# google-research/hyperbo

Measured on AMD Instinct MI355X. Metric: GP NLL+grad evals/sec at N=8192 D=16 fp64, higher is better.
Workload: dtype f64

## Files before the change

### hyperbo_amd/csrc/gemm.hip

```cpp
#include "hbo_internal.h"

namespace {

template <typename T> struct Mma;
template <> struct Mma<double> {
  typedef double acc_t __attribute__((ext_vector_type(4)));
  typedef double vec_t __attribute__((ext_vector_type(2)));
  static __device__ __forceinline__ acc_t mma(double a, double b, acc_t c) {
    return __builtin_amdgcn_mfma_f64_16x16x4f64(a, b, c, 0, 0, 0);
  }
  static __device__ __forceinline__ int crow(int lane, int r) { return (lane >> 4) + 4 * r; }
};
template <> struct Mma<float> {
  typedef float acc_t __attribute__((ext_vector_type(4)));
  typedef float vec_t __attribute__((ext_vector_type(4)));
  static __device__ __forceinline__ acc_t mma(float a, float b, acc_t c) {
    return __builtin_amdgcn_mfma_f32_16x16x4f32(a, b, c, 0, 0, 0);
  }
  static __device__ __forceinline__ int crow(int lane, int r) { return 4 * (lane >> 4) + r; }
};

template <typename T> __device__ __host__ constexpr int skc() { return sizeof(T) == 8 ? 17 : 36; }
template <int TM> __device__ __host__ constexpr int smc() { return TM + 16; }
constexpr int OPERAND_BYTES = 18432;
constexpr int OPERAND_BYTES_64 = 10240;
constexpr int GEMM_LDS_BYTES_64 = 4 * OPERAND_BYTES_64;
constexpr int GEMM_LDS_BYTES = 4 * OPERAND_BYTES;

template <typename T, bool KC, int TM>
__device__ __forceinline__ T frag_read(const T* s, int mn, int k) {
  return KC ? s[mn * skc<T>() + k] : s[k * smc<TM>() + mn];
}

template <typename T>
struct TileJob {
  const T* A; int64_t lda;
  const T* B; int64_t ldb;
  T* C; int64_t ldc;
  T* colsq;
  int ksteps;
  T alpha;
  int beta;
  int* yield_flag;
};

template <typename T, int TM>
__device__ __forceinline__ bool decode_job(const GemmArgs& g, TileJob<T>& j, const int bxi, const int byi, const int gdx, const int task) {
  constexpr int BKE = 128 / sizeof(T);
  const TaskDesc& t = g.tasks[task];
  const int64_t ld = t.ld;
  const int nblk = t.nblk;
  j.colsq = nullptr;
  switch (g.mode) {
    case GEMM_SYRK: {
      constexpr int U = HBO_TILE / TM;
      const int by = byi;
      const int bx = gridDim.z > 1 ? (int)((bxi + 5 * byi + 3 * task) % gdx) : bxi;
      const int c = g.c_lo * U + by;
      const int r = g.c_lo * U + bx;
      const int nrt = (nblk + ((g.aug & 1) ? 1 : 0)) * U;
      const int chi = (g.c_hi < nblk ? g.c_hi : nblk) * U;
      if (c >= chi || r < c || r >= nrt) return false;
      T* Am = static_cast<T*>(t.A);
      j.A = Am + (int64_t)r * TM * ld + (int64_t)g.p0 * HBO_TILE;
      j.B = Am + (int64_t)c * TM * ld + (int64_t)g.p0 * HBO_TILE;
      j.C = Am + (int64_t)r * TM * ld + (int64_t)c * TM;
      j.lda = j.ldb = j.ldc = ld;
      j.ksteps = g.kt * HBO_TILE / BKE;
      j.alpha = (T)-1; j.beta = 1;
#ifdef HBO_GEMM_DEBUG
      if (g.aug & 2) j.beta = 0;
      if (g.aug & 4) { j.C = nullptr; j.beta = 0; }
#endif
      return true;
    }
    case GEMM_TRTRI_A:
    case GEMM_TRTRI_B: {
      constexpr int U = HBO_TILE / TM;
      const int s = g.p0, su = s * U;
      const int grp = g.grp_lo + bxi / su;
      const int inner = bxi % su;
      int jt, it;
      if (g.mode == GEMM_TRTRI_A) {
        jt = byi;
        const int vu = (grp == g.c_hi ? g.c_lo : s) * U;
        it = (inner + 5 * byi + 3 * task) % vu;
      }
      else { it = (g.kt > 0 ? g.kt * U : su) - 1 - byi; jt = inner; }
      const int64_t o = (int64_t)grp * 2 * s * HBO_TILE;
      const int64_t R = o + (int64_t)s * HBO_TILE + (int64_t)it * TM;
      if (R >= (int64_t)nblk * HBO_TILE) return false;
      const int64_t Cc = o + (int64_t)jt * TM;
      const T* L = static_cast<const T*>(t.A);
      T* W = static_cast<T*>(t.W);
      T* S = static_cast<T*>(t.S);
      if (g.mode == GEMM_TRTRI_A) {
        j.A = L + R * ld + Cc;
        j.B = W + Cc * ld + Cc;
        j.C = S + R * ld + Cc;
        j.ksteps = (s * HBO_TILE - jt * TM) / BKE;
        j.alpha = (T)1;
      } else {
        const int64_t o2 = o + (int64_t)s * HBO_TILE;
        j.A = W + R * ld + o2;
        j.B = S + o2 * ld + Cc;
        j.C = W + R * ld + Cc;
        j.ksteps = (it + 1) * TM / BKE;
        j.alpha = (T)-1;
      }
      j.lda = j.ldb = j.ldc = ld;
      j.beta = 0;
      return true;
    }
    case GEMM_LAUUM: {
      constexpr int U = HBO_TILE / TM;
      int i, jt;
      if (U == 1) {
        int lin = bxi;
        if (lin >= nblk * (nblk + 1) / 2) return false;
        i = 0;
        while (lin > i) { lin -= i + 1; ++i; }
        jt = lin;
      } else {
        int lin = bxi;
        if (lin >= 2 * nblk * (nblk + 1)) return false;
        i = 0;
        while (lin > (i | 1)) { lin -= (i | 1) + 1; ++i; }
        jt = lin;
      }
      const int64_t k0 = (int64_t)i * TM;
      const T* W = static_cast<const T*>(t.W);
      j.A = W + k0 * ld + (int64_t)i * TM;
      j.B = W + k0 * ld + (int64_t)jt * TM;
      j.C = static_cast<T*>(t.S) + (int64_t)i * TM * ld + (int64_t)jt * TM;
      j.lda = j.ldb = j.ldc = ld;
      j.ksteps = (int)(((int64_t)nblk * HBO_TILE - k0) / BKE);
      j.alpha = (T)1; j.beta = 0;
      return true;
    }
    case GEMM_SWEEP_B: {
      constexpr int U = HBO_TILE / TM;
      const int b0 = g.c_lo, b1 = g.c_hi < nblk ? g.c_hi : nblk;
      const int rows = (b1 - b0) * U;
      if (byi >= rows || bxi >= b0 * U) return false;
      const int it = b0 * U + rows - 1 - byi, jt = bxi;
      const int64_t k0 = (int64_t)b0 * HBO_TILE;
      T* W = static_cast<T*>(t.W);
      j.A = W + (int64_t)it * TM * ld + k0;
      j.B = static_cast<const T*>(t.S) + k0 * ld + (int64_t)jt * TM;
      j.C = W + (int64_t)it * TM * ld + (int64_t)jt * TM;
      j.lda = j.ldb = j.ldc = ld;
      j.ksteps = (int)(((int64_t)(it + 1) * TM - k0) / BKE);
      j.alpha = (T)-1; j.beta = 0;
      return true;
    }
    case GEMM_SWEEP_T: {
      constexpr int U = HBO_TILE / TM;
      const int b0 = g.c_lo, b1 = g.c_hi;
      if (b1 >= nblk) return false;
      const int below = (nblk - b1) * U;
      const int bx = gridDim.z > 1 || g.ptasks > 1 ? (int)((bxi + 5 * byi + 3 * task) % gdx) : bxi;
      if (bx >= below || byi >= b1 * U) return false;
      const int it = b1 * U + bx, jt = byi;
      const int64_t kb = (int64_t)b0 * HBO_TILE, kj = (int64_t)jt * TM;
      const int64_t k0 = kj > kb ? kj : kb;
      j.A = static_cast<const T*>(t.A) + (int64_t)it * TM * ld + k0;
      j.B = static_cast<const T*>(t.W) + k0 * ld + kj;
      j.C = static_cast<T*>(t.S) + (int64_t)it * TM * ld + kj;
      j.lda = j.ldb = j.ldc = ld;
      j.ksteps = (int)(((int64_t)b1 * HBO_TILE - k0) / BKE);
      j.alpha = (T)1; j.beta = kj >= kb ? 0 : 1;
      return true;
    }
    case GEMM_SWEEP_C: {
      constexpr int U = HBO_TILE / TM;
      const int b0 = g.c_lo, b1 = g.c_hi < nblk ? g.c_hi : nblk;
      if (b1 <= b0) return false;
      int i = 0, lin = bxi, jt;
      if (U == 1) {
        if (lin >= b1 * (b1 + 1) / 2) return false;
        while (lin > i) { lin -= i + 1; ++i; }
      } else {
        if (lin >= 2 * b1 * (b1 + 1)) return false;
        while (lin > (i | 1)) { lin -= (i | 1) + 1; ++i; }
      }
      jt = lin;
      const int64_t kb = (int64_t)b0 * HBO_TILE, ki = (int64_t)i * TM;
      const int64_t k0 = ki > kb ? ki : kb;
      const T* W = static_cast<const T*>(t.W);
      j.A = W + k0 * ld + ki;
      j.B = W + k0 * ld + (int64_t)jt * TM;
      j.C = static_cast<T*>(t.S) + ki * ld + (int64_t)jt * TM;
      j.lda = j.ldb = j.ldc = ld;
      j.ksteps = (int)(((int64_t)b1 * HBO_TILE - k0) / BKE);
      j.alpha = (T)1; j.beta = ki >= kb ? 0 : 1;
      return true;
    }
    case GEMM_VTV: {
      const T* Vm = static_cast<const T*>(g.B);
      j.A = Vm + (int64_t)byi * HBO_TILE;
      j.B = Vm + (int64_t)bxi * HBO_TILE;
      j.C = static_cast<T*>(g.V) + (int64_t)byi * HBO_TILE * g.ldb + (int64_t)bxi * HBO_TILE;
      j.lda = j.ldb = j.ldc = g.ldb;
      j.ksteps = nblk * HBO_TILE / BKE;
      j.alpha = (T)-1; j.beta = 1;
      return true;
    }
    case GEMM_POST: {
      if (g.kchunk > 0) {
        int i = 0, rem = byi;
        for (;; ++i) {
          if (i >= nblk) return false;
          const int nch = (i + g.kchunk) / g.kchunk;
          if (rem < nch) break;
          rem -= nch;
        }
        const int k0 = rem * g.kchunk;
        const int kb = (i + 1 - k0 < g.kchunk ? i + 1 - k0 : g.kchunk);
        const T* W = static_cast<const T*>(t.W);
        j.A = W + (int64_t)i * HBO_TILE * ld + (int64_t)k0 * HBO_TILE;
        j.lda = ld;
        j.B = static_cast<const T*>(g.B) + (int64_t)k0 * HBO_TILE * g.ldb + (int64_t)bxi * HBO_TILE;
        j.ldb = g.ldb;
        j.C = static_cast<T*>(g.V) + ((int64_t)rem * nblk * HBO_TILE + (int64_t)i * HBO_TILE) * g.ldb + (int64_t)bxi * HBO_TILE;
        j.ldc = g.ldb;
        j.ksteps = kb * HBO_TILE / BKE;
        j.alpha = (T)1; j.beta = 0;
        return true;
      }
      const int i = nblk - 1 - byi;
      if (i < 0) return false;
      const int jq = bxi;
      const T* W = static_cast<const T*>(t.W);
      j.A = W + (int64_t)i * HBO_TILE * ld;
      j.lda = ld;
      j.B = static_cast<const T*>(g.B) + (int64_t)jq * HBO_TILE;
      j.ldb = g.ldb;
      j.C = g.V ? static_cast<T*>(g.V) + (int64_t)i * HBO_TILE * g.ldb + (int64_t)jq * HBO_TILE : nullptr;
      j.ldc = g.ldb;
      j.colsq = g.colsq ? static_cast<T*>(g.colsq) + (int64_t)i * g.ldb + (int64_t)jq * HBO_TILE : nullptr;
      j.ksteps = (i + 1) * HBO_TILE / BKE;
      j.alpha = (T)1; j.beta = 0;
      return true;
    }
  }
  return false;
}

template <typename T>
__device__ __forceinline__ unsigned long long uniform_addr(const T* p) {
  const unsigned long long v = reinterpret_cast<unsigned long long>(p);
  const unsigned lo = __builtin_amdgcn_readfirstlane((unsigned)v), hi = __builtin_amdgcn_readfirstlane((unsigned)(v >> 32));
  return ((unsigned long long)hi << 32) | lo;
}
__device__ __forceinline__ __amdgpu_buffer_rsrc_t tile_rsrc(unsigned long long addr) {
  return __builtin_amdgcn_make_buffer_rsrc(reinterpret_cast<void*>(addr), 0, 0x7fffffff, 0x00020000);
}
template <typename T, bool KC, int TM>
__device__ __forceinline__ void stage_offsets(int64_t ld, int (&off)[TM / 32], int tid) {
  constexpr int VEC = 16 / sizeof(T);
  if (KC) {
    const int c = tid & 7, row = tid >> 3;
#pragma unroll
    for (int q = 0; q < TM / 32; ++q) off[q] = (int)(((int64_t)(row + 32 * q) * ld + c * VEC) * (int64_t)sizeof(T));
  } else {
    constexpr int CPR = TM / VEC, RPP = 256 / CPR;
    const int c = tid % CPR, kr = tid / CPR;
#pragma unroll
    for (int q = 0; q < TM / 32; ++q) off[q] = (int)(((int64_t)(kr + RPP * q) * ld + c * VEC) * (int64_t)sizeof(T));
  }
}
template <typename T>
__device__ __forceinline__ typename Mma<T>::vec_t piece_load(unsigned long long slab, int off) {
  return __builtin_bit_cast(typename Mma<T>::vec_t, __builtin_amdgcn_raw_buffer_load_b128(tile_rsrc(slab), off, 0, 0));
}
template <typename T, bool KC, int TM>
__device__ __forceinline__ void piece_store(T* s, const typename Mma<T>::vec_t& r, int q, int tid) {
  typedef typename Mma<T>::vec_t vec_t;
  constexpr int VEC = 16 / sizeof(T);
  if (KC) {
    const int c = tid & 7, row = tid >> 3;
    if ((skc<T>() * sizeof(T)) % 16 == 0) {
      *reinterpret_cast<vec_t*>(s + (row + 32 * q) * skc<T>() + c * VEC) = r;
    } else {
#pragma unroll
      for (int e = 0; e < VEC; ++e) s[(row + 32 * q) * skc<T>() + c * VEC + e] = r[e];
    }
  } else {
    constexpr int CPR = TM / VEC, RPP = 256 / CPR;
    const int c = tid % CPR, kr = tid / CPR;
    *reinterpret_cast<vec_t*>(s + (kr + RPP * q) * smc<TM>() + c * VEC) = r;
  }
}

template <typename T, bool AKC, bool BKC, int TM>
__device__ __forceinline__ void gemm_tile2(const TileJob<T>& job, unsigned char* smem) {
  typedef typename Mma<T>::acc_t acc_t;
  typedef typename Mma<T>::vec_t vec_t;
  constexpr int BKE = 128 / sizeof(T);
  constexpr int KK = BKE / 4;
  constexpr int MI = TM / 32;
  constexpr int WT = TM / 2;
  static_assert(MI == 4 && KK >= 4 && KK % 2 == 0, "the interleave below is written for the 128-tile: 16 MFMAs and 8 fragments per k step, 8 pieces per slab");
  T* sA = reinterpret_cast<T*>(smem);
  T* sB = reinterpret_cast<T*>(smem + OPERAND_BYTES);
  const int tid = threadIdx.x, lane = tid & 63, wave = tid >> 6;
  const int wm = wave >> 1, wn = wave & 1;
  const int l15 = lane & 15, lq = lane >> 4;

  acc_t acc[MI][MI];
  if (job.beta) {
    const T inv_alpha = (T)1 / job.alpha;
#pragma unroll
    for (int a = 0; a < MI; ++a)
#pragma unroll
      for (int b = 0; b < MI; ++b)
#pragma unroll
        for (int r = 0; r < 4; ++r) {
          const int row = wm * WT + a * 16 + Mma<T>::crow(lane, r);
          const int col = wn * WT + b * 16 + l15;
          acc[a][b][r] = gld(job.C + (int64_t)row * job.ldc + col) * inv_alpha;
        }
  } else {
#pragma unroll
    for (int a = 0; a < MI; ++a)
#pragma unroll
      for (int b = 0; b < MI; ++b) acc[a][b] = (acc_t){0, 0, 0, 0};
  }

  const int nk = job.ksteps;
  int offa[MI], offb[MI];
  stage_offsets<T, AKC, TM>(job.lda, offa, tid);
  stage_offsets<T, BKC, TM>(job.ldb, offb, tid);
  unsigned long long slabA = uniform_addr(job.A), slabB = uniform_addr(job.B);
  const unsigned long long stepA = uniform_addr(reinterpret_cast<const char*>((AKC ? (int64_t)BKE : (int64_t)BKE * job.lda) * (int64_t)sizeof(T)));
  const unsigned long long stepB = uniform_addr(reinterpret_cast<const char*>((BKC ? (int64_t)BKE : (int64_t)BKE * job.ldb) * (int64_t)sizeof(T)));
  vec_t ra[MI], rb[MI];
#pragma unroll
  for (int q = 0; q < MI; ++q) { ra[q] = piece_load<T>(slabA, offa[q]); rb[q] = piece_load<T>(slabB, offb[q]); }
#pragma unroll
  for (int q = 0; q < MI; ++q) { piece_store<T, AKC, TM>(sA, ra[q], q, tid); piece_store<T, BKC, TM>(sB, rb[q], q, tid); }
  if (nk > 1) { slabA += stepA; slabB += stepB; }
#pragma unroll
  for (int q = 0; q < MI; ++q) { ra[q] = piece_load<T>(slabA, offa[q]); rb[q] = piece_load<T>(slabB, offb[q]); }
  __syncthreads();

  T af[2][MI], bf[2][MI];
#define HBO_SB() __builtin_amdgcn_sched_barrier(0)
  auto frag = [&](int set, int kk, int i) {
    const int k = kk * 4 + lq;
    if (i < MI) af[set][i] = frag_read<T, AKC, TM>(sA, wm * WT + i * 16 + l15, k);
    else bf[set][i - MI] = frag_read<T, BKC, TM>(sB, wn * WT + (i - MI) * 16 + l15, k);
  };
  auto mma = [&](int set, int i) {
    const int a = i / MI, b = (a & 1) ? MI - 1 - i % MI : i % MI;
    acc[a][b] = Mma<T>::mma(af[set][a], bf[set][b], acc[a][b]);
  };
  auto step_reads = [&](int set, int nset, int nkk) {
#pragma unroll
    for (int i = 0; i < 16; ++i) {
      mma(set, i);
      if (i < 4) { HBO_SB(); frag(nset, nkk, 2 * i); frag(nset, nkk, 2 * i + 1); HBO_SB(); }
    }
  };
  auto piece_out = [&](int j) {
    if (j < MI) piece_store<T, AKC, TM>(sA, ra[j], j, tid); else piece_store<T, BKC, TM>(sB, rb[j - MI], j - MI, tid);
  };
  auto piece_in = [&](int j) {
    if (j < MI) ra[j] = piece_load<T>(slabA, offa[j]); else rb[j - MI] = piece_load<T>(slabB, offb[j - MI]);
  };
#pragma unroll
  for (int i = 0; i < 2 * MI; ++i) frag(0, 0, i);

  const int* const yslot = job.yield_flag ? job.yield_flag + cu_token() : nullptr;
  int ypoll = 0;
  for (int kt = 0; kt + 1 < nk; ++kt) {
    if (yslot) {
      if (ypoll != 0)
        for (int spin = 0; spin < 256 && __hip_atomic_load(yslot, __ATOMIC_RELAXED, __HIP_MEMORY_SCOPE_AGENT) != 0; ++spin)
          __builtin_amdgcn_s_sleep(16);
      ypoll = __hip_atomic_load(yslot, __ATOMIC_RELAXED, __HIP_MEMORY_SCOPE_AGENT);
    }
    if (kt + 2 < nk) { slabA += stepA; slabB += stepB; }
#pragma unroll
    for (int kk = 0; kk < KK - 2; ++kk) step_reads(kk & 1, (kk + 1) & 1, kk + 1);
#pragma unroll
    for (int i = 0; i < 7; ++i) {
      mma(0, i);
      if (i < 4) { HBO_SB(); frag(1, KK - 1, 2 * i); frag(1, KK - 1, 2 * i + 1); HBO_SB(); }
    }
    HBO_SB(); __syncthreads(); HBO_SB();
    mma(0, 7);
#pragma unroll
    for (int j = 0; j < 4; ++j) {
      HBO_SB(); piece_out(j); HBO_SB(); mma(0, 8 + 2 * j); HBO_SB(); piece_in(j); HBO_SB(); mma(0, 9 + 2 * j);
    }
#pragma unroll
    for (int j = 4; j < 8; ++j) {
      HBO_SB(); piece_out(j); HBO_SB(); mma(1, 2 * (j - 4)); HBO_SB(); piece_in(j); HBO_SB(); mma(1, 2 * (j - 4) + 1);
    }
    mma(1, 8); mma(1, 9);
    HBO_SB(); __syncthreads(); HBO_SB();
    mma(1, 10);
#pragma unroll
    for (int i = 0; i < 4; ++i) { HBO_SB(); frag(0, 0, 2 * i); frag(0, 0, 2 * i + 1); HBO_SB(); mma(1, 11 + i); }
    mma(1, 15);
    HBO_SB();
  }
#pragma unroll
  for (int kk = 0; kk < KK - 1; ++kk) step_reads(kk & 1, (kk + 1) & 1, kk + 1);
#pragma unroll
  for (int i = 0; i < 16; ++i) mma(1, i);
#undef HBO_SB
  if (yslot) __syncthreads();

  if (job.C) {
#pragma unroll
    for (int a = 0; a < MI; ++a)
#pragma unroll
      for (int b = 0; b < MI; ++b)
#pragma unroll
        for (int r = 0; r < 4; ++r) {
          const int row = wm * WT + a * 16 + Mma<T>::crow(lane, r);
          const int col = wn * WT + b * 16 + l15;
          gst(job.C + (int64_t)row * job.ldc + col, job.alpha * acc[a][b][r]);
        }
  }
  if (TM == 128 && job.colsq) {
    __syncthreads();
    T* red = reinterpret_cast<T*>(smem);
    T part[MI];
#pragma unroll
    for (int b = 0; b < MI; ++b) {
      T s_ = 0;
#pragma unroll
      for (int a = 0; a < MI; ++a)
#pragma unroll
        for (int r = 0; r < 4; ++r) s_ += acc[a][b][r] * acc[a][b][r];
      s_ += __shfl_xor(s_, 16);
      s_ += __shfl_xor(s_, 32);
      part[b] = s_;
    }
    if (lq == 0) {
#pragma unroll
      for (int b = 0; b < MI; ++b) red[wave * 64 + b * 16 + l15] = part[b];
    }
    __syncthreads();
    if (tid < 128) {
      const int wn2 = tid >> 6, c = tid & 63;
      gst(job.colsq + wn2 * 64 + c, red[(0 * 2 + wn2) * 64 + c] + red[(1 * 2 + wn2) * 64 + c]);
    }
  }
}
constexpr int PF64 = 2;
constexpr int LB64 = 4;
template <typename T, bool AKC, bool BKC, int TM, int PF>
__device__ __forceinline__ void gemm_tile3(const TileJob<T>& job, unsigned char* smem) {
  typedef typename Mma<T>::acc_t acc_t;
  typedef typename Mma<T>::vec_t vec_t;
  constexpr int BKE = 128 / sizeof(T);
  constexpr int KK = BKE / 4;
  constexpr int MI = TM / 32;
  constexpr int WT = TM / 2;
  static_assert(MI == 2 && KK >= 4 && KK % 2 == 0, "written for the 64-tile: 4 MFMAs and 4 fragments per k step, 4 pieces per slab");
  T* sA = reinterpret_cast<T*>(smem);
  T* sB = reinterpret_cast<T*>(smem + OPERAND_BYTES_64);
  const int tid = threadIdx.x, lane = tid & 63, wave = tid >> 6;
  const int wm = wave >> 1, wn = wave & 1;
  const int l15 = lane & 15, lq = lane >> 4;

  acc_t acc[MI][MI];
  if (job.beta) {
    const T inv_alpha = (T)1 / job.alpha;
#pragma unroll
    for (int a = 0; a < MI; ++a)
#pragma unroll
      for (int b = 0; b < MI; ++b)
#pragma unroll
        for (int r = 0; r < 4; ++r) {
          const int row = wm * WT + a * 16 + Mma<T>::crow(lane, r);
          const int col = wn * WT + b * 16 + l15;
          acc[a][b][r] = gld(job.C + (int64_t)row * job.ldc + col) * inv_alpha;
        }
  } else {
#pragma unroll
    for (int a = 0; a < MI; ++a)
#pragma unroll
      for (int b = 0; b < MI; ++b) acc[a][b] = (acc_t){0, 0, 0, 0};
  }

  const int nk = job.ksteps;
  int offa[MI], offb[MI];
  stage_offsets<T, AKC, TM>(job.lda, offa, tid);
  stage_offsets<T, BKC, TM>(job.ldb, offb, tid);
  unsigned long long slabA = uniform_addr(job.A), slabB = uniform_addr(job.B);
  const unsigned long long stepA = uniform_addr(reinterpret_cast<const char*>((AKC ? (int64_t)BKE : (int64_t)BKE * job.lda) * (int64_t)sizeof(T)));
  const unsigned long long stepB = uniform_addr(reinterpret_cast<const char*>((BKC ? (int64_t)BKE : (int64_t)BKE * job.ldb) * (int64_t)sizeof(T)));
  vec_t ra[PF][MI], rb[PF][MI];
  auto fetch = [&](int set) {
#pragma unroll
    for (int q = 0; q < MI; ++q) { ra[set][q] = piece_load<T>(slabA, offa[q]); rb[set][q] = piece_load<T>(slabB, offb[q]); }
    slabA += stepA; slabB += stepB;
  };
  auto to_lds = [&](int set) {
#pragma unroll
    for (int q = 0; q < MI; ++q) { piece_store<T, AKC, TM>(sA, ra[set][q], q, tid); piece_store<T, BKC, TM>(sB, rb[set][q], q, tid); }
  };
#pragma unroll
  for (int u = 0; u < PF; ++u)
    if (u < nk) fetch(u);
  to_lds(0);
  if (PF < nk) fetch(0);
  __syncthreads();

  T af[2][MI], bf[2][MI];
#define HBO_SB() __builtin_amdgcn_sched_barrier(0)
  auto frags = [&](int set, int kk) {
    const int k = kk * 4 + lq;
#pragma unroll
    for (int a = 0; a < MI; ++a) af[set][a] = frag_read<T, AKC, TM>(sA, wm * WT + a * 16 + l15, k);
#pragma unroll
    for (int b = 0; b < MI; ++b) bf[set][b] = frag_read<T, BKC, TM>(sB, wn * WT + b * 16 + l15, k);
  };
  auto mma = [&](int set, int i) {
    const int a = i / MI, b = (a & 1) ? MI - 1 - i % MI : i % MI;
    acc[a][b] = Mma<T>::mma(af[set][a], bf[set][b], acc[a][b]);
  };
  auto step = [&](int set, int nset, int nkk) {
    mma(set, 0); HBO_SB(); frags(nset, nkk); HBO_SB(); mma(set, 1); mma(set, 2); mma(set, 3);
  };
  frags(0, 0);

  const int* const yslot = job.yield_flag ? job.yield_flag + cu_token() : nullptr;
  int ypoll = 0;
  for (int s0 = 0; s0 + 1 < nk; s0 += PF) {
#pragma unroll
    for (int u = 0; u < PF; ++u) {
      const int s = s0 + u;
      if (s + 1 >= nk) break;
      const int set = (u + 1) % PF;
      if (yslot) {
        if (ypoll != 0)
          for (int spin = 0; spin < 256 && __hip_atomic_load(yslot, __ATOMIC_RELAXED, __HIP_MEMORY_SCOPE_AGENT) != 0; ++spin)
            __builtin_amdgcn_s_sleep(16);
        ypoll = __hip_atomic_load(yslot, __ATOMIC_RELAXED, __HIP_MEMORY_SCOPE_AGENT);
      }
#pragma unroll
      for (int kk = 0; kk < KK - 2; ++kk) step(kk & 1, (kk + 1) & 1, kk + 1);
      mma(0, 0); HBO_SB(); frags(1, KK - 1); HBO_SB(); mma(0, 1);
      HBO_SB(); __syncthreads(); HBO_SB();
      mma(0, 2); HBO_SB(); to_lds(set); HBO_SB(); mma(0, 3);
      if (s + 1 + PF < nk) fetch(set);
      mma(1, 0); mma(1, 1);
      HBO_SB(); __syncthreads(); HBO_SB();
      mma(1, 2); HBO_SB(); frags(0, 0); HBO_SB(); mma(1, 3);
    }
  }
#pragma unroll
  for (int kk = 0; kk < KK - 1; ++kk) step(kk & 1, (kk + 1) & 1, kk + 1);
  mma(1, 0); mma(1, 1); mma(1, 2); mma(1, 3);
#undef HBO_SB

  if (job.C) {
#pragma unroll
    for (int a = 0; a < MI; ++a)
#pragma unroll
      for (int b = 0; b < MI; ++b)
#pragma unroll
        for (int r = 0; r < 4; ++r) {
          const int row = wm * WT + a * 16 + Mma<T>::crow(lane, r);
          const int col = wn * WT + b * 16 + l15;
          gst(job.C + (int64_t)row * job.ldc + col, job.alpha * acc[a][b][r]);
        }
  }
}
template <typename T, bool AKC, bool BKC, int TM>
__device__ __forceinline__ void run_tile(const TileJob<T>& job, unsigned char* smem) {
  if constexpr (TM == 128) gemm_tile2<T, AKC, BKC, TM>(job, smem);
  else gemm_tile3<T, AKC, BKC, TM, PF64>(job, smem);
}

template <typename T, int TM>
__device__ __forceinline__ bool decode_syrk_linear(const GemmArgs& g, int tix, TileJob<T>& j) {
  constexpr int BKE = 128 / sizeof(T);
  constexpr int U = HBO_TILE / TM;
  const TaskDesc& t = g.tasks[blockIdx.z];
  const int nblk = t.nblk;
  const int nrt = (nblk + ((g.aug & 1) ? 1 : 0)) * U;
  const int chi = (g.c_hi < nblk ? g.c_hi : nblk) * U;
  int c = g.c_lo * U;
  while (c < chi && tix >= nrt - c) { tix -= nrt - c; ++c; }
  if (c >= chi) return false;
  const int r = c + tix;
  const int64_t ld = t.ld;
  T* Am = static_cast<T*>(t.A);
  j.A = Am + (int64_t)r * TM * ld + (int64_t)g.p0 * HBO_TILE;
  j.B = Am + (int64_t)c * TM * ld + (int64_t)g.p0 * HBO_TILE;
  j.C = Am + (int64_t)r * TM * ld + (int64_t)c * TM;
  j.lda = j.ldb = j.ldc = ld;
  j.colsq = nullptr;
  j.ksteps = g.kt * HBO_TILE / BKE;
  j.alpha = (T)-1; j.beta = 1;
  return true;
}

#ifdef HBO_GEMM_TIMING
__device__ unsigned long long hbo_dbg_gemm[4 * 8192];
int g_dbg_mode = -1, g_dbg_index = 0, g_dbg_seen = 0;
#endif
template <typename T, bool AKC, bool BKC, int TM>
__device__ __forceinline__ void gemm_kernel_body(const GemmArgs& g, unsigned char* smem) {
  TileJob<T> job;
  job.yield_flag = g.yield_flag;
#ifdef HBO_GEMM_TIMING
  const int dbg_id = blockIdx.y * gridDim.x + blockIdx.x;
  const bool dbg = g.dbg && blockIdx.z == 0 && dbg_id < 8192 && threadIdx.x == 0;
  if (dbg) {
    hbo_dbg_gemm[4 * dbg_id] = wall_clock64();
    hbo_dbg_gemm[4 * dbg_id + 1] = 0;
    hbo_dbg_gemm[4 * dbg_id + 2] = ((unsigned long long)__builtin_amdgcn_s_getreg((20 << 0) | (0 << 6) | (31 << 11)) << 32) |
                                   (unsigned)__builtin_amdgcn_s_getreg((4 << 0) | (0 << 6) | (31 << 11));
    hbo_dbg_gemm[4 * dbg_id + 3] = 0;
  }
#endif
  if (AKC && BKC && g.persistent) {
#ifdef HBO_GEMM_TIMING
    unsigned long long dbg_ks = 0;
#endif
    __shared__ int s_tix;
    for (int tix = blockIdx.x;; tix += gridDim.x) {
      if (g.work_counter) {
        if (threadIdx.x == 0) s_tix = atomicAdd(g.work_counter, 1);
        __syncthreads();
        tix = s_tix;
        __syncthreads();
      }
      if (TM == 128 && g.n_big > 0 && tix >= g.n_big) {
        const int s4 = tix - g.n_big;
        if (!decode_syrk_linear<T, 128>(g, g.n_big + (s4 >> 2), job)) break;
        const int qr = (s4 >> 1) & 1, qc = s4 & 1;
        const int64_t ldq = job.lda;
        job.A += (int64_t)qr * 64 * ldq;
        job.B += (int64_t)qc * 64 * ldq;
        job.C += (int64_t)qr * 64 * ldq + qc * 64;
        run_tile<T, AKC, BKC, 64>(job, smem);
        continue;
      }
      if (!decode_syrk_linear<T, TM>(g, tix, job)) break;
      run_tile<T, AKC, BKC, TM>(job, smem);
#ifdef HBO_GEMM_TIMING
      dbg_ks += (unsigned long long)job.ksteps;
#endif
    }
#ifdef HBO_GEMM_TIMING
    if (dbg) { hbo_dbg_gemm[4 * dbg_id + 1] = wall_clock64(); hbo_dbg_gemm[4 * dbg_id + 3] = dbg_ks; }
#endif
    return;
  }
  if (!(AKC && BKC) && g.persistent) {
    __shared__ int s_tix2;
    const int nt = g.ptasks > 1 ? g.ptasks : 1;
    const int total = g.pgx * g.pgy * nt;
    for (;;) {
      if (threadIdx.x == 0) s_tix2 = atomicAdd(g.work_counter, 1);
      __syncthreads();
      const int tix = s_tix2;
      __syncthreads();
      if (tix >= total) break;
      const int tile = tix / nt, task = g.ptasks > 1 ? tix % nt : (int)blockIdx.z;
      if (decode_job<T, TM>(g, job, tile % g.pgx, tile / g.pgx, g.pgx, task)) run_tile<T, AKC, BKC, TM>(job, smem);
    }
    return;
  }
  if (!decode_job<T, TM>(g, job, (int)blockIdx.x, (int)blockIdx.y, (int)gridDim.x, (int)blockIdx.z)) return;
  int ytok = 0;
  if (g.yield_mark && threadIdx.x == 0) ytok = yield_enter(g.yield_mark);
  run_tile<T, AKC, BKC, TM>(job, smem);
  if (g.yield_mark) {
    __syncthreads();
    if (threadIdx.x == 0) yield_leave(g.yield_mark, ytok);
  }
#ifdef HBO_GEMM_TIMING
  if (dbg) { hbo_dbg_gemm[4 * dbg_id + 1] = wall_clock64(); hbo_dbg_gemm[4 * dbg_id + 3] = (unsigned long long)job.ksteps; }
#endif
}

template <typename T, bool AKC, bool BKC, int TM>
__global__ __launch_bounds__(256, TM == 64 ? LB64 : 2) void gemm_kernel(GemmArgs g) {
  extern __shared__ __attribute__((aligned(16))) unsigned char smem[];
  tl_begin(g.tl);
  gemm_kernel_body<T, AKC, BKC, TM>(g, smem);
  tl_end(g.tl);
}

enum Operands { OPS_KK, OPS_KM, OPS_MM };
enum TileGrid {
  TILES_XY,
  TILES_TRI,
};
struct ModeRow {
  Operands ops;
  TileGrid tiles;
  bool tiles64;
  bool resident;
  bool needs_counter;
  bool one_task;
  bool only128;
  bool over_tasks;
};
constexpr ModeRow MODE_TABLE[] = {
   {OPS_KK, TILES_XY,  true,  true,  false, false, false, false},
   {OPS_KM, TILES_XY,  true,  true,  true,  true,  false, false},
   {OPS_KM, TILES_XY,  true,  true,  true,  true,  false, false},
   {OPS_MM, TILES_TRI, true,  true,  true,  true,  true,  false},
   {OPS_KM, TILES_XY,  false, true,  true,  true,  false, false},
   {OPS_MM, TILES_XY,  false, false, false, false, false, false},
   {OPS_KM, TILES_XY,  true,  true,  true,  false, false, true},
   {OPS_KM, TILES_XY,  true,  true,  true,  false, false, true},
   {OPS_MM, TILES_TRI, true,  true,  true,  false, false, true},
};
constexpr int N_MODES = sizeof(MODE_TABLE) / sizeof(ModeRow);
static_assert(GEMM_SYRK == 0 && GEMM_TRTRI_A == 1 && GEMM_TRTRI_B == 2 && GEMM_LAUUM == 3 && GEMM_POST == 4 && GEMM_VTV == 5 &&
              GEMM_SWEEP_B == 6 && GEMM_SWEEP_T == 7 && GEMM_SWEEP_C == 8 && N_MODES == 9, "one row per GemmMode, in its order");

constexpr int LDS_64 = GEMM_LDS_BYTES_64;
constexpr int LDS_128 = 2 * OPERAND_BYTES > LDS_64 ? 2 * OPERAND_BYTES : LDS_64;

struct GemmPlan { GemmArgs a; Operands ops; int tm; dim3 grid; int lds; };
GemmPlan gemm_plan(const GemmArgs& a_in, dim3 grid) {
  const ModeRow& row = MODE_TABLE[a_in.mode];
  GemmPlan p = {a_in, row.ops, row.tiles64 && a_in.small_tiles ? 64 : 128, grid, 0};
  GemmArgs& a = p.a;
  const bool resident_ok = row.resident && (!row.needs_counter || a.work_counter) && (!row.one_task || grid.z == 1) && (!row.only128 || p.tm == 128);
  if (!resident_ok || a.persistent <= 0) { a.persistent = 0; a.work_counter = nullptr; }
  const unsigned u = p.tm == 64 ? 2 : 1, n = grid.x;
  const dim3 tiles = row.tiles == TILES_TRI ? dim3(u == 2 ? 2 * n * (n + 1) : n * (n + 1) / 2, 1, grid.z) : dim3(grid.x * u, grid.y * u, grid.z);
  a.ptasks = 0;
  if (a.persistent > 0) {
    if (row.ops != OPS_KK) { a.pgx = (int)tiles.x; a.pgy = (int)tiles.y; }
    if (row.over_tasks) a.ptasks = (int)grid.z;
    p.grid = dim3(a.persistent, 1, row.over_tasks ? 1 : grid.z);
  } else {
    p.grid = tiles;
  }
  p.lds = p.tm == 64 ? LDS_64 : LDS_128;
  return p;
}

template <typename T, bool AKC, bool BKC>
void launch_plan(const GemmPlan& p, hipStream_t st) {
  if (p.tm == 64) hipLaunchKernelGGL((gemm_kernel<T, AKC, BKC, 64>), p.grid, dim3(256), p.lds, st, p.a);
  else hipLaunchKernelGGL((gemm_kernel<T, AKC, BKC, 128>), p.grid, dim3(256), p.lds, st, p.a);
}
template <typename T>
void launch_gemm_t(const GemmArgs& a, dim3 grid, hipStream_t st) {
  static unsigned long long attr_seen = 0;
  if (hbo_first_use_on_device(attr_seen)) {
    hipFuncSetAttribute(reinterpret_cast<const void*>(&gemm_kernel<T, true, true, 128>),
                        hipFuncAttributeMaxDynamicSharedMemorySize, GEMM_LDS_BYTES);
    hipFuncSetAttribute(reinterpret_cast<const void*>(&gemm_kernel<T, true, false, 128>),
                        hipFuncAttributeMaxDynamicSharedMemorySize, GEMM_LDS_BYTES);
    hipFuncSetAttribute(reinterpret_cast<const void*>(&gemm_kernel<T, false, false, 128>),
                        hipFuncAttributeMaxDynamicSharedMemorySize, GEMM_LDS_BYTES);
  }
  if (a.mode < 0 || a.mode >= N_MODES) return;
  const GemmPlan p = gemm_plan(a, grid);
  switch (p.ops) {
    case OPS_KK: launch_plan<T, true, true>(p, st); break;
    case OPS_KM: launch_plan<T, true, false>(p, st); break;
    case OPS_MM: launch_plan<T, false, false>(p, st); break;
  }
}

}

#ifdef HBO_GEMM_TIMING
extern "C" void hbo_dbg_gemm_wall(unsigned long long* host, int mode, int index) {
  if (host) { hipMemcpyFromSymbol(host, HIP_SYMBOL(hbo_dbg_gemm), sizeof(unsigned long long) * 4 * 8192); return; }
  static unsigned long long zeros[4 * 8192];
  hipMemcpyToSymbol(HIP_SYMBOL(hbo_dbg_gemm), zeros, sizeof zeros);
  g_dbg_mode = mode; g_dbg_index = index; g_dbg_seen = 0;
}
#endif
void launch_gemm(int dtype, const GemmArgs& a_in, dim3 grid, hipStream_t st) {
  GemmArgs a = a_in;
#ifdef HBO_GEMM_TIMING
  a.dbg = 0;
  if ((a.persistent ? a.mode + 100 : a.mode) == g_dbg_mode) a.dbg = (g_dbg_seen++ == g_dbg_index);
#endif
  if (dtype == HBO_F64) launch_gemm_t<double>(a, grid, st);
  else launch_gemm_t<float>(a, grid, st);
}
```

Measured before the change: 93.73.

## Keep persistent SYRK tiles resident and prefetch the next tile during the k-loop

Turns the tile GEMM into a reusable struct so that a persistent SYRK walker can draw the next tile's work index early, redirect the operand slabs to the next tile near the end of the current k-loop, and defer the previous tile's C store so it overlaps the next tile's staging. C loads and stores now go through buffer intrinsics with uniform scalar offsets instead of per-element global address arithmetic. The aim is to hide the per-tile prologue and epilogue bubbles (atomic draw, first slab loads, sync) between consecutive persistent tiles. It adds more live state and register pressure, changes the ordering of the work-counter draws, and adds optional phase-timing instrumentation.

```diff
diff --git a/hyperbo_amd/csrc/gemm.hip b/hyperbo_amd/csrc/gemm.hip
--- a/hyperbo_amd/csrc/gemm.hip
+++ b/hyperbo_amd/csrc/gemm.hip
@@ -253,6 +253,8 @@
   const unsigned lo = __builtin_amdgcn_readfirstlane((unsigned)v), hi = __builtin_amdgcn_readfirstlane((unsigned)(v >> 32));
   return ((unsigned long long)hi << 32) | lo;
 }
+__device__ __forceinline__ int uniform_int(int v) { return __builtin_amdgcn_readfirstlane(v); }
+__device__ __forceinline__ int64_t uniform_i64(int64_t v) { return (int64_t)uniform_addr(reinterpret_cast<const char*>(v)); }
 __device__ __forceinline__ __amdgpu_buffer_rsrc_t tile_rsrc(unsigned long long addr) {
   return __builtin_amdgcn_make_buffer_rsrc(reinterpret_cast<void*>(addr), 0, 0x7fffffff, 0x00020000);
 }
@@ -273,6 +275,21 @@
 template <typename T>
 __device__ __forceinline__ typename Mma<T>::vec_t piece_load(unsigned long long slab, int off) {
   return __builtin_bit_cast(typename Mma<T>::vec_t, __builtin_amdgcn_raw_buffer_load_b128(tile_rsrc(slab), off, 0, 0));
+}
+template <typename T> __device__ __forceinline__ T c_load(__amdgpu_buffer_rsrc_t rs, int voff, int soff);
+template <> __device__ __forceinline__ double c_load<double>(__amdgpu_buffer_rsrc_t rs, int voff, int soff) {
+  return __builtin_bit_cast(double, __builtin_amdgcn_raw_buffer_load_b64(rs, voff, soff, 0));
+}
+template <> __device__ __forceinline__ float c_load<float>(__amdgpu_buffer_rsrc_t rs, int voff, int soff) {
+  return __builtin_bit_cast(float, __builtin_amdgcn_raw_buffer_load_b32(rs, voff, soff, 0));
+}
+template <typename T> __device__ __forceinline__ void c_store(T v, __amdgpu_buffer_rsrc_t rs, int voff, int soff);
+template <> __device__ __forceinline__ void c_store<double>(double v, __amdgpu_buffer_rsrc_t rs, int voff, int soff) {
+  typedef unsigned u2 __attribute__((ext_vector_type(2)));
+  __builtin_amdgcn_raw_buffer_store_b64(__builtin_bit_cast(u2, v), rs, voff, soff, 0);
+}
+template <> __device__ __forceinline__ void c_store<float>(float v, __amdgpu_buffer_rsrc_t rs, int voff, int soff) {
+  __builtin_amdgcn_raw_buffer_store_b32(__builtin_bit_cast(unsigned, v), rs, voff, soff, 0);
 }
 template <typename T, bool KC, int TM>
 __device__ __forceinline__ void piece_store(T* s, const typename Mma<T>::vec_t& r, int q, int tid) {
@@ -293,140 +310,193 @@
   }
 }
 
+enum TilePhase { PH_DRAW, PH_STAGE, PH_STORE_C, PH_LOAD_C, PH_SYNC, PH_K_FIRST, PH_K_REST, PH_TAIL, N_PHASES };
+#ifdef HBO_GEMM_TIMING
+struct PhaseClock {
+  unsigned long long ph[N_PHASES], last;
+  __device__ __forceinline__ void start() {
+#pragma unroll
+    for (int k = 0; k < N_PHASES; ++k) ph[k] = 0;
+    last = wall_clock64();
+  }
+  __device__ __forceinline__ void mark(int k) { const unsigned long long n = wall_clock64(); ph[k] += n - last; last = n; }
+};
+#else
+struct PhaseClock {
+  __device__ __forceinline__ void start() {}
+  __device__ __forceinline__ void mark(int) {}
+};
+#endif
+
+struct NoNext {
+  static constexpr bool ahead = false;
+  unsigned long long A = 0, B = 0;
+  __device__ __forceinline__ void publish() {}
+  __device__ __forceinline__ bool resolve() { return false; }
+};
+
 template <typename T, bool AKC, bool BKC, int TM>
-__device__ __forceinline__ void gemm_tile2(const TileJob<T>& job, unsigned char* smem) {
+struct Tile2 {
   typedef typename Mma<T>::acc_t acc_t;
   typedef typename Mma<T>::vec_t vec_t;
-  constexpr int BKE = 128 / sizeof(T);
-  constexpr int KK = BKE / 4;
-  constexpr int MI = TM / 32;
-  constexpr int WT = TM / 2;
+  static constexpr int BKE = 128 / sizeof(T);
+  static constexpr int KK = BKE / 4;
+  static constexpr int MI = TM / 32;
+  static constexpr int WT = TM / 2;
   static_assert(MI == 4 && KK >= 4 && KK % 2 == 0, "the interleave below is written for the 128-tile: 16 MFMAs and 8 fragments per k step, 8 pieces per slab");
-  T* sA = reinterpret_cast<T*>(smem);
-  T* sB = reinterpret_cast<T*>(smem + OPERAND_BYTES);
-  const int tid = threadIdx.x, lane = tid & 63, wave = tid >> 6;
-  const int wm = wave >> 1, wn = wave & 1;
-  const int l15 = lane & 15, lq = lane >> 4;
-
+  T* sA; T* sB;
+  int tid, lane, wave, wm, wn, l15, lq;
   acc_t acc[MI][MI];
-  if (job.beta) {
-    const T inv_alpha = (T)1 / job.alpha;
-#pragma unroll
-    for (int a = 0; a < MI; ++a)
-#pragma unroll
-      for (int b = 0; b < MI; ++b)
-#pragma unroll
-        for (int r = 0; r < 4; ++r) {
-          const int row = wm * WT + a * 16 + Mma<T>::crow(lane, r);
-          const int col = wn * WT + b * 16 + l15;
-          acc[a][b][r] = gld(job.C + (int64_t)row * job.ldc + col) * inv_alpha;
-        }
-  } else {
-#pragma unroll
-    for (int a = 0; a < MI; ++a)
-#pragma unroll
-      for (int b = 0; b < MI; ++b) acc[a][b] = (acc_t){0, 0, 0, 0};
-  }
-
-  const int nk = job.ksteps;
+  vec_t ra[MI], rb[MI];
+  T af[2][MI], bf[2][MI];
   int offa[MI], offb[MI];
-  stage_offsets<T, AKC, TM>(job.lda, offa, tid);
-  stage_offsets<T, BKC, TM>(job.ldb, offb, tid);
-  unsigned long long slabA = uniform_addr(job.A), slabB = uniform_addr(job.B);
-  const unsigned long long stepA = uniform_addr(reinterpret_cast<const char*>((AKC ? (int64_t)BKE : (int64_t)BKE * job.lda) * (int64_t)sizeof(T)));
-  const unsigned long long stepB = uniform_addr(reinterpret_cast<const char*>((BKC ? (int64_t)BKE : (int64_t)BKE * job.ldb) * (int64_t)sizeof(T)));
-  vec_t ra[MI], rb[MI];
-#pragma unroll
-  for (int q = 0; q < MI; ++q) { ra[q] = piece_load<T>(slabA, offa[q]); rb[q] = piece_load<T>(slabB, offb[q]); }
-#pragma unroll
-  for (int q = 0; q < MI; ++q) { piece_store<T, AKC, TM>(sA, ra[q], q, tid); piece_store<T, BKC, TM>(sB, rb[q], q, tid); }
-  if (nk > 1) { slabA += stepA; slabB += stepB; }
-#pragma unroll
-  for (int q = 0; q < MI; ++q) { ra[q] = piece_load<T>(slabA, offa[q]); rb[q] = piece_load<T>(slabB, offb[q]); }
-  __syncthreads();
-
-  T af[2][MI], bf[2][MI];
-#define HBO_SB() __builtin_amdgcn_sched_barrier(0)
-  auto frag = [&](int set, int kk, int i) {
+  unsigned long long slabA, slabB, stepA, stepB;
+  const int* yslot;
+
+  __device__ __forceinline__ Tile2(unsigned char* smem, int* yield_flag) {
+    sA = reinterpret_cast<T*>(smem);
+    sB = reinterpret_cast<T*>(smem + OPERAND_BYTES);
+    tid = threadIdx.x; lane = tid & 63; wave = tid >> 6;
+    wm = wave >> 1; wn = wave & 1;
+    l15 = lane & 15; lq = lane >> 4;
+    yslot = yield_flag ? yield_flag + cu_token() : nullptr;
+  }
+  __device__ __forceinline__ int c_pitch(int64_t ldc) const { return uniform_int((int)(ldc * (int64_t)sizeof(T))); }
+  __device__ __forceinline__ int c_lane_offset(int64_t ldc) const {
+    return (int)(((int64_t)(wm * WT + Mma<T>::crow(lane, 0)) * ldc + wn * WT + l15) * (int64_t)sizeof(T));
+  }
+  __device__ __forceinline__ void load_c(const TileJob<T>& job) {
+    if (job.beta) {
+      const T inv_alpha = (T)1 / job.alpha;
+      const __amdgpu_buffer_rsrc_t rs = tile_rsrc(uniform_addr(job.C));
+      const int pitch = c_pitch(job.ldc), voff = c_lane_offset(job.ldc);
+#pragma unroll
+      for (int a = 0; a < MI; ++a)
+#pragma unroll
+        for (int b = 0; b < MI; ++b)
+#pragma unroll
+          for (int r = 0; r < 4; ++r)
+            acc[a][b][r] = c_load<T>(rs, voff + b * 16 * (int)sizeof(T), (a * 16 + Mma<T>::crow(0, r)) * pitch) * inv_alpha;
+    } else {
+#pragma unroll
+      for (int a = 0; a < MI; ++a)
+#pragma unroll
+        for (int b = 0; b < MI; ++b) acc[a][b] = (acc_t){0, 0, 0, 0};
+    }
+  }
+  __device__ __forceinline__ void strides(int64_t lda, int64_t ldb) {
+    stage_offsets<T, AKC, TM>(lda, offa, tid);
+    stage_offsets<T, BKC, TM>(ldb, offb, tid);
+    stepA = uniform_addr(reinterpret_cast<const char*>((AKC ? (int64_t)BKE : (int64_t)BKE * lda) * (int64_t)sizeof(T)));
+    stepB = uniform_addr(reinterpret_cast<const char*>((BKC ? (int64_t)BKE : (int64_t)BKE * ldb) * (int64_t)sizeof(T)));
+  }
+  __device__ __forceinline__ void load_first(const TileJob<T>& job) {
+    slabA = uniform_addr(job.A); slabB = uniform_addr(job.B);
+#pragma unroll
+    for (int q = 0; q < MI; ++q) { ra[q] = piece_load<T>(slabA, offa[q]); rb[q] = piece_load<T>(slabB, offb[q]); }
+  }
+  __device__ __forceinline__ void stage(int nk) {
+#pragma unroll
+    for (int q = 0; q < MI; ++q) { piece_store<T, AKC, TM>(sA, ra[q], q, tid); piece_store<T, BKC, TM>(sB, rb[q], q, tid); }
+    if (nk > 1) { slabA += stepA; slabB += stepB; }
+#pragma unroll
+    for (int q = 0; q < MI; ++q) { ra[q] = piece_load<T>(slabA, offa[q]); rb[q] = piece_load<T>(slabB, offb[q]); }
+  }
+  __device__ __forceinline__ void frag(int set, int kk, int i) {
     const int k = kk * 4 + lq;
     if (i < MI) af[set][i] = frag_read<T, AKC, TM>(sA, wm * WT + i * 16 + l15, k);
     else bf[set][i - MI] = frag_read<T, BKC, TM>(sB, wn * WT + (i - MI) * 16 + l15, k);
-  };
-  auto mma = [&](int set, int i) {
+  }
+  __device__ __forceinline__ void first_frags() {
+    __syncthreads();
+#pragma unroll
+    for (int i = 0; i < 2 * MI; ++i) frag(0, 0, i);
+  }
+  __device__ __forceinline__ void mma(int set, int i) {
     const int a = i / MI, b = (a & 1) ? MI - 1 - i % MI : i % MI;
     acc[a][b] = Mma<T>::mma(af[set][a], bf[set][b], acc[a][b]);
-  };
-  auto step_reads = [&](int set, int nset, int nkk) {
+  }
+#define HBO_SB() __builtin_amdgcn_sched_barrier(0)
+  __device__ __forceinline__ void step_reads(int set, int nset, int nkk) {
 #pragma unroll
     for (int i = 0; i < 16; ++i) {
       mma(set, i);
       if (i < 4) { HBO_SB(); frag(nset, nkk, 2 * i); frag(nset, nkk, 2 * i + 1); HBO_SB(); }
     }
-  };
-  auto piece_out = [&](int j) {
+  }
+  __device__ __forceinline__ void piece_out(int j) {
     if (j < MI) piece_store<T, AKC, TM>(sA, ra[j], j, tid); else piece_store<T, BKC, TM>(sB, rb[j - MI], j - MI, tid);
-  };
-  auto piece_in = [&](int j) {
+  }
+  __device__ __forceinline__ void piece_in(int j) {
     if (j < MI) ra[j] = piece_load<T>(slabA, offa[j]); else rb[j - MI] = piece_load<T>(slabB, offb[j - MI]);
-  };
-#pragma unroll
-  for (int i = 0; i < 2 * MI; ++i) frag(0, 0, i);
-
-  const int* const yslot = job.yield_flag ? job.yield_flag + cu_token() : nullptr;
-  int ypoll = 0;
-  for (int kt = 0; kt + 1 < nk; ++kt) {
-    if (yslot) {
-      if (ypoll != 0)
-        for (int spin = 0; spin < 256 && __hip_atomic_load(yslot, __ATOMIC_RELAXED, __HIP_MEMORY_SCOPE_AGENT) != 0; ++spin)
-          __builtin_amdgcn_s_sleep(16);
-      ypoll = __hip_atomic_load(yslot, __ATOMIC_RELAXED, __HIP_MEMORY_SCOPE_AGENT);
-    }
-    if (kt + 2 < nk) { slabA += stepA; slabB += stepB; }
-#pragma unroll
-    for (int kk = 0; kk < KK - 2; ++kk) step_reads(kk & 1, (kk + 1) & 1, kk + 1);
-#pragma unroll
-    for (int i = 0; i < 7; ++i) {
-      mma(0, i);
-      if (i < 4) { HBO_SB(); frag(1, KK - 1, 2 * i); frag(1, KK - 1, 2 * i + 1); HBO_SB(); }
-    }
-    HBO_SB(); __syncthreads(); HBO_SB();
-    mma(0, 7);
-#pragma unroll
-    for (int j = 0; j < 4; ++j) {
-      HBO_SB(); piece_out(j); HBO_SB(); mma(0, 8 + 2 * j); HBO_SB(); piece_in(j); HBO_SB(); mma(0, 9 + 2 * j);
-    }
-#pragma unroll
-    for (int j = 4; j < 8; ++j) {
-      HBO_SB(); piece_out(j); HBO_SB(); mma(1, 2 * (j - 4)); HBO_SB(); piece_in(j); HBO_SB(); mma(1, 2 * (j - 4) + 1);
-    }
-    mma(1, 8); mma(1, 9);
-    HBO_SB(); __syncthreads(); HBO_SB();
-    mma(1, 10);
-#pragma unroll
-    for (int i = 0; i < 4; ++i) { HBO_SB(); frag(0, 0, 2 * i); frag(0, 0, 2 * i + 1); HBO_SB(); mma(1, 11 + i); }
-    mma(1, 15);
-    HBO_SB();
-  }
-#pragma unroll
-  for (int kk = 0; kk < KK - 1; ++kk) step_reads(kk & 1, (kk + 1) & 1, kk + 1);
-#pragma unroll
-  for (int i = 0; i < 16; ++i) mma(1, i);
+  }
+  template <typename Next>
+  __device__ __forceinline__ bool kloop(const int nk, Next& next, PhaseClock& clk) {
+    int ypoll = 0;
+    bool more = false;
+    for (int kt = 0; kt + 1 < nk; ++kt) {
+      if (yslot) {
+        if (ypoll != 0)
+          for (int spin = 0; spin < 256 && __hip_atomic_load(yslot, __ATOMIC_RELAXED, __HIP_MEMORY_SCOPE_AGENT) != 0; ++spin)
+            __builtin_amdgcn_s_sleep(16);
+        ypoll = __hip_atomic_load(yslot, __ATOMIC_RELAXED, __HIP_MEMORY_SCOPE_AGENT);
+      }
+      if (Next::ahead && kt == 1) next.publish();
+      if (kt + 2 < nk) { slabA += stepA; slabB += stepB; }
+      else if (Next::ahead) {
+        more = next.resolve();
+        if (more) { slabA = next.A; slabB = next.B; }
+      }
+#pragma unroll
+      for (int kk = 0; kk < KK - 2; ++kk) step_reads(kk & 1, (kk + 1) & 1, kk + 1);
+#pragma unroll
+      for (int i = 0; i < 7; ++i) {
+        mma(0, i);
+        if (i < 4) { HBO_SB(); frag(1, KK - 1, 2 * i); frag(1, KK - 1, 2 * i + 1); HBO_SB(); }
+      }
+      HBO_SB(); __syncthreads(); HBO_SB();
+      mma(0, 7);
+#pragma unroll
+      for (int j = 0; j < 4; ++j) {
+        HBO_SB(); piece_out(j); HBO_SB(); mma(0, 8 + 2 * j); HBO_SB(); piece_in(j); HBO_SB(); mma(0, 9 + 2 * j);
+      }
+#pragma unroll
+      for (int j = 4; j < 8; ++j) {
+        HBO_SB(); piece_out(j); HBO_SB(); mma(1, 2 * (j - 4)); HBO_SB(); piece_in(j); HBO_SB(); mma(1, 2 * (j - 4) + 1);
+      }
+      mma(1, 8); mma(1, 9);
+      HBO_SB(); __syncthreads(); HBO_SB();
+      mma(1, 10);
+#pragma unroll
+      for (int i = 0; i < 4; ++i) { HBO_SB(); frag(0, 0, 2 * i); frag(0, 0, 2 * i + 1); HBO_SB(); mma(1, 11 + i); }
+      mma(1, 15);
+      HBO_SB();
+#ifdef HBO_GEMM_TIMING
+      if (kt == 0) clk.mark(PH_K_FIRST);
+#endif
+    }
+#pragma unroll
+    for (int kk = 0; kk < KK - 1; ++kk) step_reads(kk & 1, (kk + 1) & 1, kk + 1);
+#pragma unroll
+    for (int i = 0; i < 16; ++i) mma(1, i);
+    clk.mark(PH_K_REST);
+    return more;
+  }
 #undef HBO_SB
-  if (yslot) __syncthreads();
-
-  if (job.C) {
-#pragma unroll
-    for (int a = 0; a < MI; ++a)
-#pragma unroll
-      for (int b = 0; b < MI; ++b)
-#pragma unroll
-        for (int r = 0; r < 4; ++r) {
-          const int row = wm * WT + a * 16 + Mma<T>::crow(lane, r);
-          const int col = wn * WT + b * 16 + l15;
-          gst(job.C + (int64_t)row * job.ldc + col, job.alpha * acc[a][b][r]);
-        }
-  }
-  if (TM == 128 && job.colsq) {
+  __device__ __forceinline__ void store_c(T* C, int64_t ldc, T alpha) {
+    if (C) {
+      const __amdgpu_buffer_rsrc_t rs = tile_rsrc(uniform_addr(C));
+      const int pitch = c_pitch(ldc), voff = c_lane_offset(ldc);
+#pragma unroll
+      for (int a = 0; a < MI; ++a)
+#pragma unroll
+        for (int b = 0; b < MI; ++b)
+#pragma unroll
+          for (int r = 0; r < 4; ++r)
+            c_store<T>(alpha * acc[a][b][r], rs, voff + b * 16 * (int)sizeof(T), (a * 16 + Mma<T>::crow(0, r)) * pitch);
+    }
+  }
+  __device__ __forceinline__ void store_colsq(T* colsq, unsigned char* smem) {
     __syncthreads();
     T* red = reinterpret_cast<T*>(smem);
     T part[MI];
@@ -448,9 +518,26 @@
     __syncthreads();
     if (tid < 128) {
       const int wn2 = tid >> 6, c = tid & 63;
-      gst(job.colsq + wn2 * 64 + c, red[(0 * 2 + wn2) * 64 + c] + red[(1 * 2 + wn2) * 64 + c]);
-    }
-  }
+      gst(colsq + wn2 * 64 + c, red[(0 * 2 + wn2) * 64 + c] + red[(1 * 2 + wn2) * 64 + c]);
+    }
+  }
+};
+
+template <typename T, bool AKC, bool BKC, int TM>
+__device__ __forceinline__ void gemm_tile2(const TileJob<T>& job, unsigned char* smem) {
+  Tile2<T, AKC, BKC, TM> t(smem, job.yield_flag);
+  PhaseClock clk;
+  clk.start();
+  NoNext none;
+  t.load_c(job);
+  t.strides(job.lda, job.ldb);
+  t.load_first(job);
+  t.stage(job.ksteps);
+  t.first_frags();
+  t.kloop(job.ksteps, none, clk);
+  if (t.yslot) __syncthreads();
+  t.store_c(job.C, job.ldc, job.alpha);
+  if (TM == 128 && job.colsq) t.store_colsq(job.colsq, smem);
 }
 constexpr int PF64 = 2;
 constexpr int LB64 = 4;
@@ -604,8 +691,107 @@
   return true;
 }
 
+
+template <typename T>
+struct SyrkWalk {
+  static constexpr bool ahead = true;
+  const GemmArgs& g;
+  int* slot;
+  int nrt, chi, limit;
+  int64_t ld;
+  T* Am;
+  int c, base;
+  int tix;
+  int drawn;
+  TileJob<T> job;
+  unsigned long long A, B;
+
+  __device__ __forceinline__ SyrkWalk(const GemmArgs& g_, int* slot_) : g(g_), slot(slot_) {
+    const TaskDesc& t = g.tasks[blockIdx.z];
+    const int nblk = uniform_int(t.nblk);
+    ld = uniform_i64(t.ld);
+    Am = reinterpret_cast<T*>(uniform_addr(static_cast<T*>(t.A)));
+    nrt = nblk + ((g.aug & 1) ? 1 : 0);
+    chi = g.c_hi < nblk ? g.c_hi : nblk;
+    limit = g.n_big > 0 ? g.n_big : 0x7fffffff;
+    c = g.c_lo; base = 0; tix = 0; drawn = 0;
+    job.lda = job.ldb = job.ldc = ld;
+    job.colsq = nullptr;
+    job.ksteps = g.kt * HBO_TILE / (128 / (int)sizeof(T));
+    job.alpha = (T)-1; job.beta = 1;
+    job.yield_flag = g.yield_flag;
+  }
+  __device__ __forceinline__ int first() {
+    int t = blockIdx.x;
+    if (g.work_counter) {
+      if (threadIdx.x == 0) *slot = atomicAdd(g.work_counter, 1);
+      __syncthreads();
+      t = *slot;
+      __syncthreads();
+    }
+    return uniform_int(t);
+  }
+  __device__ __forceinline__ bool decode(int t) {
+    tix = t;
+    if (t >= limit) return false;
+    while (c < chi && t - base >= nrt - c) { base += nrt - c; ++c; }
+    if (c >= chi) return false;
+    const int r = c + (t - base);
+    job.A = Am + (int64_t)r * HBO_TILE * ld + (int64_t)g.p0 * HBO_TILE;
+    job.B = Am + (int64_t)c * HBO_TILE * ld + (int64_t)g.p0 * HBO_TILE;
+    job.C = Am + (int64_t)r * HBO_TILE * ld + (int64_t)c * HBO_TILE;
+    A = uniform_addr(job.A); B = uniform_addr(job.B);
+    return true;
+  }
+  __device__ __forceinline__ void issue() {
+    if (g.work_counter) {
+      if (threadIdx.x == 0) drawn = atomicAdd(g.work_counter, 1);
+    } else {
+      drawn = tix + (int)gridDim.x;
+    }
+  }
+  __device__ __forceinline__ void publish() {
+    if (g.work_counter && threadIdx.x == 0) *slot = drawn;
+  }
+  __device__ __forceinline__ bool resolve() { return decode(uniform_int(g.work_counter ? *slot : drawn)); }
+};
+
+template <typename T, bool AKC, bool BKC, typename Walk>
+__device__ __forceinline__ void gemm_resident(Walk& w, unsigned char* smem, PhaseClock& clk, unsigned long long& ksteps) {
+  Tile2<T, AKC, BKC, 128> t(smem, w.job.yield_flag);
+  TileJob<T> job = w.job;
+  T* c_prev = nullptr;
+  int64_t ld_prev = 0;
+  T alpha_prev = (T)0;
+  bool prev = false;
+  t.strides(job.lda, job.ldb);
+  t.load_first(job);
+  for (;;) {
+    const int nk = job.ksteps;
+    ksteps += (unsigned long long)nk;
+    w.issue();
+    clk.mark(PH_DRAW);
+    t.stage(nk);
+    clk.mark(PH_STAGE);
+    if (prev) t.store_c(c_prev, ld_prev, alpha_prev);
+    clk.mark(PH_STORE_C);
+    t.load_c(job);
+    clk.mark(PH_LOAD_C);
+    t.first_frags();
+    clk.mark(PH_SYNC);
+    if (!t.kloop(nk, w, clk)) break;
+    __syncthreads();
+    c_prev = job.C; ld_prev = job.ldc; alpha_prev = job.alpha; prev = true;
+    job = w.job;
+    clk.mark(PH_SYNC);
+  }
+  t.store_c(job.C, job.ldc, job.alpha);
+  clk.mark(PH_STORE_C);
+}
+
 #ifdef HBO_GEMM_TIMING
 __device__ unsigned long long hbo_dbg_gemm[4 * 8192];
+__device__ unsigned long long hbo_dbg_phase[N_PHASES * 8192];
 int g_dbg_mode = -1, g_dbg_index = 0, g_dbg_seen = 0;
 #endif
 template <typename T, bool AKC, bool BKC, int TM>
@@ -624,36 +810,52 @@
   }
 #endif
   if (AKC && BKC && g.persistent) {
+    __shared__ int s_tix;
+    PhaseClock clk;
+    clk.start();
+    unsigned long long dbg_ks = 0;
+    int tix = blockIdx.x;
+    bool have = !g.work_counter;
+    if constexpr (TM == 128) {
+      SyrkWalk<T> w(g, &s_tix);
+      if (w.decode(w.first())) gemm_resident<T, AKC, BKC>(w, smem, clk, dbg_ks);
+      tix = w.tix; have = true;
+      if (g.n_big > 0) __syncthreads();
+    }
+    if (TM == 64 || g.n_big > 0) {
+      for (;; have = false) {
+        if (!have) {
+          if (g.work_counter) {
+            if (threadIdx.x == 0) s_tix = atomicAdd(g.work_counter, 1);
+            __syncthreads();
+            tix = s_tix;
+            __syncthreads();
+          } else {
+            tix += gridDim.x;
+          }
+        }
+        if constexpr (TM == 128) {
+          const int s4 = tix - g.n_big;
+          if (!decode_syrk_linear<T, 128>(g, g.n_big + (s4 >> 2), job)) break;
+          const int qr = (s4 >> 1) & 1, qc = s4 & 1;
+          const int64_t ldq = job.lda;
+          job.A += (int64_t)qr * 64 * ldq;
+          job.B += (int64_t)qc * 64 * ldq;
+          job.C += (int64_t)qr * 64 * ldq + qc * 64;
+        } else {
+          if (!decode_syrk_linear<T, TM>(g, tix, job)) break;
+          dbg_ks += (unsigned long long)job.ksteps;
+        }
+        run_tile<T, AKC, BKC, 64>(job, smem);
+      }
+    }
+    clk.mark(PH_TAIL);
 #ifdef HBO_GEMM_TIMING
-    unsigned long long dbg_ks = 0;
-#endif
-    __shared__ int s_tix;
-    for (int tix = blockIdx.x;; tix += gridDim.x) {
-      if (g.work_counter) {
-        if (threadIdx.x == 0) s_tix = atomicAdd(g.work_counter, 1);
-        __syncthreads();
-        tix = s_tix;
-        __syncthreads();
-      }
-      if (TM == 128 && g.n_big > 0 && tix >= g.n_big) {
-        const int s4 = tix - g.n_big;
-        if (!decode_syrk_linear<T, 128>(g, g.n_big + (s4 >> 2), job)) break;
-        const int qr = (s4 >> 1) & 1, qc = s4 & 1;
-        const int64_t ldq = job.lda;
-        job.A += (int64_t)qr * 64 * ldq;
-        job.B += (int64_t)qc * 64 * ldq;
-        job.C += (int64_t)qr * 64 * ldq + qc * 64;
-        run_tile<T, AKC, BKC, 64>(job, smem);
-        continue;
-      }
-      if (!decode_syrk_linear<T, TM>(g, tix, job)) break;
-      run_tile<T, AKC, BKC, TM>(job, smem);
-#ifdef HBO_GEMM_TIMING
-      dbg_ks += (unsigned long long)job.ksteps;
-#endif
-    }
-#ifdef HBO_GEMM_TIMING
-    if (dbg) { hbo_dbg_gemm[4 * dbg_id + 1] = wall_clock64(); hbo_dbg_gemm[4 * dbg_id + 3] = dbg_ks; }
+    if (dbg) {
+      hbo_dbg_gemm[4 * dbg_id + 1] = wall_clock64(); hbo_dbg_gemm[4 * dbg_id + 3] = dbg_ks;
+#pragma unroll
+      for (int k = 0; k < N_PHASES; ++k) hbo_dbg_phase[N_PHASES * dbg_id + k] = clk.ph[k];
+    }
 #endif
     return;
   }
@@ -776,6 +978,7 @@
 
 #ifdef HBO_GEMM_TIMING
 extern "C" void hbo_dbg_gemm_wall(unsigned long long* host, int mode, int index) {
+  if (host && mode == -2) { hipMemcpyFromSymbol(host, HIP_SYMBOL(hbo_dbg_phase), sizeof(unsigned long long) * N_PHASES * 8192); return; }
   if (host) { hipMemcpyFromSymbol(host, HIP_SYMBOL(hbo_dbg_gemm), sizeof(unsigned long long) * 4 * 8192); return; }
   static unsigned long long zeros[4 * 8192];
   hipMemcpyToSymbol(HIP_SYMBOL(hbo_dbg_gemm), zeros, sizeof zeros);
```

After: 94.41, median of 6. About the same (+0.7%).
